# agentmorris/MegaDetector

Hardware: AMD Instinct MI355X
Metric: images/sec (whole node) MDv5a @1280px batch inference (higher is better)
Workload: dtype bf16

## Files before the change

### megadetector_amd/csrc/conv_v5c.cpp

```cpp

#include <algorithm>
#include <cstdlib>
#include <type_traits>

#include "mdhip_internal.h"

namespace mdhip {
namespace MDHIP_ST {

namespace {

typedef __attribute__((ext_vector_type(4))) float f32x4;
typedef __attribute__((address_space(3))) char lds_char;

[[maybe_unused]] constexpr unsigned kOOB = 0x80000000u;
[[maybe_unused]] constexpr int kNumRecords = 0x7fffffff;

__device__ __forceinline__ float silu_f32(float x) {
    return x * __builtin_amdgcn_rcpf(1.0f + __expf(-x));
}

constexpr int kPixB = 160;
constexpr int c80_run_bytes(int bm) { return ((bm + 2) * kPixB + 1023) & ~1023; }
constexpr int kW1Bytes = 9 * 80 * 32;
constexpr int c80_zero_bytes(int fm) { return ((15 + fm * 16 + 2) * kPixB + 32 + 255) & ~255; }
constexpr int c80_lds_bytes(int bm, int wm) { return 4 * c80_run_bytes(bm) + kW1Bytes + c80_zero_bytes(bm / (16 * wm)) + 320 + 1024; }
constexpr int c80f_lds_bytes(int bm, int wm) { return c80_lds_bytes(bm, wm) + 80 * 192 + 320; }
constexpr int c80_blocks(int bm, int wm) { return 163840 / c80_lds_bytes(bm, wm) >= 2 && wm == 1 ? 2 : 1; }

}

#define MDHIP_DMA16(rsrc, lptr, voff, soff) \
    __builtin_amdgcn_raw_ptr_buffer_load_lds((rsrc), (lptr), 16, (voff), (soff), 0, 0)

template <int BM, int WM>
__global__ void __launch_bounds__(WM * 5 * 64, c80_blocks(BM, WM))
conv_c80_kernel(const ConvArgs p) {
#if defined(__HIP_DEVICE_COMPILE__)
    constexpr int kNWc = WM * 5;
    constexpr int FM = BM / (16 * WM);
    constexpr int RUNB = c80_run_bytes(BM), PIECES = RUNB / 1024, NP = (PIECES + kNWc - 1) / kNWc;
    constexpr int W1_OFF = 4 * RUNB, ZERO_OFF = W1_OFF + kW1Bytes, BIAS_OFF = ZERO_OFF + c80_zero_bytes(FM);
    constexpr int SCRATCH_OFF = BIAS_OFF + 320;

    extern __shared__ __attribute__((aligned(16))) char smem_generic[];
    lds_char* const smem = (lds_char*)smem_generic;
    const int tid = threadIdx.x;
    const int lane = tid & 63;
    const int wave = __builtin_amdgcn_readfirstlane(tid >> 6);
    const int wm = wave / 5, wn = wave - 5 * wm;
    const int m15 = lane & 15, kb = lane >> 4;

    const int strips = p.tiles_n, segs = p.tiles_per_xcd, seg_rows = p.m_streams, total = p.tiles_m;
    const int xcd = blockIdx.x & 7, slot = blockIdx.x >> 3, slots = gridDim.x >> 3;
    const int per_xcd = (total + 7) / 8;
    const int u_lo = xcd * per_xcd, u_hi = min(u_lo + per_xcd, total);
    if (u_lo + slot >= u_hi) return;

    for (int c = tid * 16; c < c80_zero_bytes(FM); c += kNWc * 64 * 16)
        *(__attribute__((address_space(3))) uint4*)(smem + ZERO_OFF + c) = make_uint4(0, 0, 0, 0);
    for (int c = tid; c < 80; c += kNWc * 64) *(__attribute__((address_space(3))) float*)(smem + BIAS_OFF + c * 4) = p.bias[c];
    for (int c = tid; c < 9 * 80 * 2; c += kNWc * 64) {
        const int t = c / 160, rem = c - t * 160, ch = rem >> 1, half = rem & 1;
        *(__attribute__((address_space(3))) uint4*)(smem + W1_OFF + c * 16) =
            *(const uint4*)(p.wgt4 + (size_t)ch * p.k_pad4 + (9 + t) * 64 + half * 8);
    }
    frag8_t wreg[9][2];
#pragma unroll
    for (int t = 0; t < 9; ++t)
#pragma unroll
        for (int kk = 0; kk < 2; ++kk)
            wreg[t][kk] = *(const frag8_t*)(p.wgt4 + (size_t)(wn * 16 + m15) * p.k_pad4 + t * 64 + kk * 32 + kb * 8);
    const f32x4 bias4 = {p.bias[wn * 16 + kb * 4], p.bias[wn * 16 + kb * 4 + 1], p.bias[wn * 16 + kb * 4 + 2],
                         p.bias[wn * 16 + kb * 4 + 3]};

    int l_px[NP];
    unsigned l_off[NP], l_dst[NP];
#pragma unroll
    for (int k = 0; k < NP; ++k) {
        const int pc = wave + kNWc * k;
        const int g = pc * 64 + lane;
        const int px = g / 10, c16 = g - px * 10;
        l_px[k] = (pc < PIECES && px < BM + 2) ? px : 0x40000000;
        l_off[k] = (unsigned)((px * p.ld_in + c16 * 8) * 2);
        l_dst[k] = pc < PIECES ? (unsigned)(pc * 1024) : (unsigned)(SCRATCH_OFF - 0);
    }
    __amdgpu_buffer_rsrc_t in_rsrc, res_rsrc, out_rsrc;
    const int img_in_bytes = p.HoWo * p.ld_in * 2, img_out_bytes = p.HoWo * p.ld_out * 2, img_res_bytes = p.HoWo * p.ld_res * 2;
    int x0 = 0;
    auto issue_row = [&](int iy) __attribute__((always_inline)) {
        const unsigned sl = (unsigned)(((iy + 1) & 3) * RUNB);
        const bool row_ok = (unsigned)iy < (unsigned)p.H;
        const unsigned row_term = (unsigned)((iy * p.W + x0 - 1) * p.ld_in * 2);
#pragma unroll
        for (int k = 0; k < NP; ++k) {
            const bool ok = row_ok && (unsigned)(x0 - 1 + l_px[k]) < (unsigned)p.W;
            MDHIP_DMA16(in_rsrc, smem + (l_dst[k] >= (unsigned)SCRATCH_OFF ? l_dst[k] : sl + l_dst[k]), ok ? row_term + l_off[k] : kOOB, 0);
        }
    };

    const unsigned lane_a = (unsigned)((wm * (BM / WM) + m15) * kPixB + kb * 16);
    const unsigned lane_a1 = kb < 2 ? lane_a + 128u : 0xffffffffu;
    const unsigned lane_z = (unsigned)(ZERO_OFF + m15 * kPixB + (kb & 1) * 16);
    const unsigned lane_w1 = kb < 2 ? (unsigned)(W1_OFF + (wn * 16 + m15) * 32 + kb * 16) : (unsigned)ZERO_OFF;
    const unsigned lane_w1_step = kb < 2 ? 80u * 32u : 0u;

    f32x4 acc[FM];
#pragma unroll
    for (int i = 0; i < FM; ++i) acc[i] = f32x4{0.f, 0.f, 0.f, 0.f};

    bool first = true;
    for (int u = u_lo + slot; u < u_hi; u += slots) {
        const int xs = u % strips;
        const int t2 = u / strips;
        const int sg = t2 % segs, b = t2 / segs;
        x0 = xs * BM;
        const int y_lo = sg * seg_rows, y_hi = min(y_lo + seg_rows, p.H);
        in_rsrc = __builtin_amdgcn_make_buffer_rsrc((void*)(p.in + (size_t)b * p.HoWo * p.ld_in), 0, img_in_bytes, 0x00020000);
        out_rsrc = __builtin_amdgcn_make_buffer_rsrc((void*)((char*)p.out + (size_t)b * img_out_bytes), 0, img_out_bytes, 0x00020000);
        if (p.res)
            res_rsrc = __builtin_amdgcn_make_buffer_rsrc((void*)(p.res + (size_t)b * p.HoWo * p.ld_res), 0, img_res_bytes, 0x00020000);
        if (!first) __builtin_amdgcn_s_barrier();
        issue_row(y_lo - 1);
        issue_row(y_lo);
        issue_row(y_lo + 1);
        const int xw = x0 + wm * (BM / WM) + m15;
        for (int y = y_lo; y < y_hi; ++y) {
            if (first || y == y_lo) asm volatile("s_waitcnt vmcnt(0) lgkmcnt(0)" ::: "memory");
            else asm volatile("s_waitcnt vmcnt(%0)" ::"n"(FM) : "memory");
            first = false;
            __builtin_amdgcn_s_barrier();
            if (y + 1 < y_hi) issue_row(y + 2);
            typedef __attribute__((ext_vector_type(2))) unsigned u32x2;
            u32x2 rres[FM];
            if (p.res) {
#pragma unroll
                for (int i = 0; i < FM; ++i) {
                    const int x = xw + i * 16;
                    const unsigned off = x < p.W ? (unsigned)(((y * p.W + x) * p.ld_res + wn * 16 + kb * 4) * 2) : kOOB;
                    rres[i] = __builtin_amdgcn_raw_buffer_load_b64(res_rsrc, off, 0, 0);
                }
            }
            unsigned rb[3], rb1[3];
#pragma unroll
            for (int r = 0; r < 3; ++r) {
                const unsigned s0 = (unsigned)(((y + r) & 3) * RUNB);
                rb[r] = s0 + lane_a;
                rb1[r] = kb < 2 ? s0 + lane_a1 : lane_z;
            }
#pragma unroll
            for (int hs = 0; hs < 27; ++hs) {
                frag8_t xa[FM], w;
                if (hs < 18) {
                    const int t = hs >> 1, kk = hs & 1, r = t / 3, s = t - 3 * r;
#pragma unroll
                    for (int i = 0; i < FM; ++i)
                        xa[i] = *(const __attribute__((address_space(3))) frag8_t*)(smem + rb[r] + (i * 16 + s) * kPixB + kk * 64);
                    w = wreg[t][kk];
                } else {
                    const int t = hs - 18, r = t / 3, s = t - 3 * r;
#pragma unroll
                    for (int i = 0; i < FM; ++i)
                        xa[i] = *(const __attribute__((address_space(3))) frag8_t*)(smem + rb1[r] + (i * 16 + s) * kPixB);
                    w = *(const __attribute__((address_space(3))) frag8_t*)(smem + lane_w1 + t * lane_w1_step);
                }
#pragma unroll
                for (int i = 0; i < FM; ++i) acc[i] = MDHIP_MFMA(w, xa[i], acc[i]);
            }
#pragma unroll
            for (int i = 0; i < FM; ++i) {
                float v[4];
                mdhip_bias4(acc[i], bias4, v);
                if (p.act) mdhip_silu4(v);
                acc[i] = f32x4{0.f, 0.f, 0.f, 0.f};
                if (p.res) {
                    v[0] += st_unpack((uint16_t)(rres[i][0] & 0xffff));
                    v[1] += st_unpack((uint16_t)(rres[i][0] >> 16));
                    v[2] += st_unpack((uint16_t)(rres[i][1] & 0xffff));
                    v[3] += st_unpack((uint16_t)(rres[i][1] >> 16));
                }
                const u32x2 d = {st_pack2(v[0], v[1]), st_pack2(v[2], v[3])};
                const int x = xw + i * 16;
                const unsigned off = x < p.W ? (unsigned)(((y * p.W + x) * p.ld_out + wn * 16 + kb * 4) * 2) : kOOB;
                __builtin_amdgcn_raw_buffer_store_b64(d, out_rsrc, off, 0, 0);
            }
        }
    }
#endif
}

template <int BM, int WM>
__global__ void __launch_bounds__(WM * 5 * 64, 1)
conv_c80f_kernel(const ConvArgs p) {
#if defined(__HIP_DEVICE_COMPILE__)
    constexpr int kNWc = WM * 5;
    constexpr int FM = BM / (16 * WM);
    constexpr int RUNB = c80_run_bytes(BM), PIECES = RUNB / 1024, NP = (PIECES + kNWc - 1) / kNWc;
    constexpr int STAGE_OFF = 3 * RUNB;
    constexpr int W1_OFF = 4 * RUNB, ZERO_OFF = W1_OFF + kW1Bytes, BIAS_OFF = ZERO_OFF + c80_zero_bytes(FM);
    constexpr int SCRATCH_OFF = BIAS_OFF + 320;
    constexpr int WPRE_OFF = SCRATCH_OFF + 1024;
    constexpr int BPRE_OFF = WPRE_OFF + 80 * 192;
    constexpr int TF = (BM + 2 + 15) / 16;
    constexpr int TFW = (TF + WM - 1) / WM;
    static_assert(((TFW - 1) * 16 + 15) * kPixB + 16 <= c80_zero_bytes(FM) + 0, "zero region covers the conversion's immediates");

    extern __shared__ __attribute__((aligned(16))) char smem_generic[];
    lds_char* const smem = (lds_char*)smem_generic;
    const int tid = threadIdx.x;
    const int lane = tid & 63;
    const int wave = __builtin_amdgcn_readfirstlane(tid >> 6);
    const int wm = wave / 5, wn = wave - 5 * wm;
    const int m15 = lane & 15, kb = lane >> 4;

    const int strips = p.tiles_n, segs = p.tiles_per_xcd, seg_rows = p.m_streams, total = p.tiles_m;
    const int xcd = blockIdx.x & 7, slot = blockIdx.x >> 3, slots = gridDim.x >> 3;
    const int per_xcd = (total + 7) / 8;
    const int u_lo = xcd * per_xcd, u_hi = min(u_lo + per_xcd, total);
    if (u_lo + slot >= u_hi) return;

    for (int c = tid * 16; c < c80_zero_bytes(FM); c += kNWc * 64 * 16)
        *(__attribute__((address_space(3))) uint4*)(smem + ZERO_OFF + c) = make_uint4(0, 0, 0, 0);
    for (int c = tid; c < 9 * 80 * 2; c += kNWc * 64) {
        const int t = c / 160, rem = c - t * 160, ch = rem >> 1, half = rem & 1;
        *(__attribute__((address_space(3))) uint4*)(smem + W1_OFF + c * 16) =
            *(const uint4*)(p.wgt4 + (size_t)ch * p.k_pad4 + (9 + t) * 64 + half * 8);
    }
    frag8_t wreg[9][2];
#pragma unroll
    for (int t = 0; t < 9; ++t)
#pragma unroll
        for (int kk = 0; kk < 2; ++kk)
            wreg[t][kk] = *(const frag8_t*)(p.wgt4 + (size_t)(wn * 16 + m15) * p.k_pad4 + t * 64 + kk * 32 + kb * 8);
    for (int c = tid; c < 80 * 12; c += kNWc * 64) {
        const int ch = c / 12, q = c - ch * 12;
        *(__attribute__((address_space(3))) uint4*)(smem + WPRE_OFF + c * 16) = *(const uint4*)(p.wgt_pre + (size_t)ch * p.k_pad_pre + q * 8);
    }
    for (int c = tid; c < 80; c += kNWc * 64) *(__attribute__((address_space(3))) float*)(smem + BPRE_OFF + c * 4) = p.bias_pre[c];
    const unsigned lane_wp = (unsigned)(WPRE_OFF + (wn * 16 + m15) * 192 + kb * 16);
    const f32x4 bias4 = {p.bias[wn * 16 + kb * 4], p.bias[wn * 16 + kb * 4 + 1], p.bias[wn * 16 + kb * 4 + 2],
                         p.bias[wn * 16 + kb * 4 + 3]};

    __amdgpu_buffer_rsrc_t in_rsrc, res_rsrc, out_rsrc;
    const int img_in_bytes = p.HoWo * p.ld_in * 2, img_out_bytes = p.HoWo * p.ld_out * 2, img_res_bytes = p.HoWo * p.ld_res * 2;
    int x0 = 0;
    auto issue_row = [&](int iy) __attribute__((always_inline)) {
        const bool row_ok = (unsigned)iy < (unsigned)p.H;
        const unsigned row_term = (unsigned)((iy * p.W + x0 - 1) * p.ld_in * 2);
#pragma unroll
        for (int k = 0; k < NP; ++k) {
            const int pc = wave + kNWc * k;
            const int g = pc * 64 + lane;
            const int px = g / 10, c16 = g - px * 10;
            const bool ok = row_ok && pc < PIECES && px < BM + 2 && (unsigned)(x0 - 1 + px) < (unsigned)p.W;
            MDHIP_DMA16(in_rsrc, smem + (pc < PIECES ? STAGE_OFF + pc * 1024 : SCRATCH_OFF),
                        ok ? row_term + (unsigned)((px * p.ld_in + c16 * 8) * 2) : kOOB, 0);
        }
    };

    const unsigned lane_a = (unsigned)((wm * (BM / WM) + m15) * kPixB + kb * 16);
    const unsigned lane_a1 = kb < 2 ? lane_a + 128u : 0xffffffffu;
    const unsigned lane_z = (unsigned)(ZERO_OFF + m15 * kPixB + (kb & 1) * 16);
    const unsigned lane_w1 = kb < 2 ? (unsigned)(W1_OFF + (wn * 16 + m15) * 32 + kb * 16) : (unsigned)ZERO_OFF;
    const unsigned lane_w1_step = kb < 2 ? 80u * 32u : 0u;
    const unsigned lane_x = (unsigned)(STAGE_OFF + (wm * TFW * 16 + m15) * kPixB + kb * 16);
    const unsigned lane_x2 = kb < 2 ? lane_x + 128u : lane_z;
    const unsigned lane_t = (unsigned)((wm * TFW * 16 + m15) * kPixB + (wn * 16 + kb * 4) * 2);

    f32x4 acc[FM];
#pragma unroll
    for (int i = 0; i < FM; ++i) acc[i] = f32x4{0.f, 0.f, 0.f, 0.f};

    auto convert = [&](int iy, int ts) __attribute__((always_inline)) {
        const bool row_ok = (unsigned)iy < (unsigned)p.H;
        frag8_t wp[3];
#pragma unroll
        for (int t = 0; t < 3; ++t) wp[t] = *(const __attribute__((address_space(3))) frag8_t*)(smem + lane_wp + t * 64);
        const f32x4 bpre4 = *(const __attribute__((address_space(3))) f32x4*)(smem + BPRE_OFF + (wn * 16 + kb * 4) * 4);
#pragma unroll
        for (int f = 0; f < TFW; ++f) {
            if (wm * TFW + f < TF) {
                f32x4 c = {0.f, 0.f, 0.f, 0.f};
#pragma unroll
                for (int t = 0; t < 3; ++t) {
                    const frag8_t xf = *(const __attribute__((address_space(3))) frag8_t*)(smem + (t < 2 ? lane_x + t * 64 : lane_x2) + f * 16 * kPixB);
                    c = MDHIP_MFMA(wp[t], xf, c);
                }
                const int px = (wm * TFW + f) * 16 + m15;
                const bool ok = row_ok && px < BM + 2 && (unsigned)(x0 - 1 + px) < (unsigned)p.W;
                float v[4];
                mdhip_bias4(c, bpre4, v);
                mdhip_silu4(v);
                uint2 d;
                d.x = ok ? st_pack2(v[0], v[1]) : 0u;
                d.y = ok ? st_pack2(v[2], v[3]) : 0u;
                if (px < BM + 2)
                    *(__attribute__((address_space(3))) uint2*)(smem + ts * RUNB + lane_t + f * 16 * kPixB) = d;
            }
        }
    };

    bool first = true;
    for (int u = u_lo + slot; u < u_hi; u += slots) {
        const int xs = u % strips;
        const int t2 = u / strips;
        const int sg = t2 % segs, b = t2 / segs;
        x0 = xs * BM;
        const int y_lo = sg * seg_rows, y_hi = min(y_lo + seg_rows, p.H);
        in_rsrc = __builtin_amdgcn_make_buffer_rsrc((void*)(p.in + (size_t)b * p.HoWo * p.ld_in), 0, img_in_bytes, 0x00020000);
        out_rsrc = __builtin_amdgcn_make_buffer_rsrc((void*)((char*)p.out + (size_t)b * img_out_bytes), 0, img_out_bytes, 0x00020000);
        if (p.res)
            res_rsrc = __builtin_amdgcn_make_buffer_rsrc((void*)(p.res + (size_t)b * p.HoWo * p.ld_res), 0, img_res_bytes, 0x00020000);
        for (int k = 0; k < 3; ++k) {
            if (!first || k > 0) __builtin_amdgcn_s_barrier();
            first = false;
            issue_row(y_lo - 1 + k);
            asm volatile("s_waitcnt vmcnt(0) lgkmcnt(0)" ::: "memory");
            __builtin_amdgcn_s_barrier();
            convert(y_lo - 1 + k, k);
        }
        asm volatile("s_waitcnt lgkmcnt(0)" ::: "memory");
        __builtin_amdgcn_s_barrier();
        if (y_lo + 1 < y_hi) issue_row(y_lo + 2);
        const int xw = x0 + wm * (BM / WM) + m15;
        int s0 = 0;
        for (int y = y_lo; y < y_hi; ++y) {
            typedef __attribute__((ext_vector_type(2))) unsigned u32x2;
            u32x2 rres[FM];
            if (p.res) {
#pragma unroll
                for (int i = 0; i < FM; ++i) {
                    const int x = xw + i * 16;
                    const unsigned off = x < p.W ? (unsigned)(((y * p.W + x) * p.ld_res + wn * 16 + kb * 4) * 2) : kOOB;
                    rres[i] = __builtin_amdgcn_raw_buffer_load_b64(res_rsrc, off, 0, 0);
                }
            }
            unsigned rb[3], rb1[3];
#pragma unroll
            for (int r = 0; r < 3; ++r) {
                int sl = s0 + r;
                sl = sl >= 3 ? sl - 3 : sl;
                rb[r] = (unsigned)(sl * RUNB) + lane_a;
                rb1[r] = kb < 2 ? (unsigned)(sl * RUNB) + lane_a1 : lane_z;
            }
#pragma unroll
            for (int hs = 0; hs < 27; ++hs) {
                frag8_t xa[FM], w;
                if (hs < 18) {
                    const int t = hs >> 1, kk = hs & 1, r = t / 3, s = t - 3 * r;
#pragma unroll
                    for (int i = 0; i < FM; ++i)
                        xa[i] = *(const __attribute__((address_space(3))) frag8_t*)(smem + rb[r] + (i * 16 + s) * kPixB + kk * 64);
                    w = wreg[t][kk];
                } else {
                    const int t = hs - 18, r = t / 3, s = t - 3 * r;
#pragma unroll
                    for (int i = 0; i < FM; ++i)
                        xa[i] = *(const __attribute__((address_space(3))) frag8_t*)(smem + rb1[r] + (i * 16 + s) * kPixB);
                    w = *(const __attribute__((address_space(3))) frag8_t*)(smem + lane_w1 + t * lane_w1_step);
                }
#pragma unroll
                for (int i = 0; i < FM; ++i) acc[i] = MDHIP_MFMA(w, xa[i], acc[i]);
            }
#pragma unroll
            for (int i = 0; i < FM; ++i) {
                float v[4];
                mdhip_bias4(acc[i], bias4, v);
                if (p.act) mdhip_silu4(v);
                acc[i] = f32x4{0.f, 0.f, 0.f, 0.f};
                if (p.res) {
                    v[0] += st_unpack((uint16_t)(rres[i][0] & 0xffff));
                    v[1] += st_unpack((uint16_t)(rres[i][0] >> 16));
                    v[2] += st_unpack((uint16_t)(rres[i][1] & 0xffff));
                    v[3] += st_unpack((uint16_t)(rres[i][1] >> 16));
                }
                const u32x2 d = {st_pack2(v[0], v[1]), st_pack2(v[2], v[3])};
                const int x = xw + i * 16;
                const unsigned off = x < p.W ? (unsigned)(((y * p.W + x) * p.ld_out + wn * 16 + kb * 4) * 2) : kOOB;
                __builtin_amdgcn_raw_buffer_store_b64(d, out_rsrc, off, 0, 0);
            }
            if (y + 1 < y_hi) {
                asm volatile("s_waitcnt vmcnt(%0) lgkmcnt(0)" ::"n"(FM) : "memory");
                __builtin_amdgcn_s_barrier();
                convert(y + 2, s0);
                asm volatile("s_waitcnt lgkmcnt(0)" ::: "memory");
                __builtin_amdgcn_s_barrier();
                if (y + 2 < y_hi) issue_row(y + 3);
                s0 = s0 == 2 ? 0 : s0 + 1;
            }
        }
    }
#endif
}

constexpr int kD_BM = 64, kD_RW = 4, kD_RUNB = c80_run_bytes(kD_BM), kD_RING = kD_RW + 2;
constexpr int kD_STAGE_OFF = kD_RING * kD_RUNB, kD_W1_OFF = kD_STAGE_OFF + kD_RW * kD_RUNB, kD_ZERO_OFF = kD_W1_OFF + kW1Bytes;
constexpr int kD_WPRE_OFF = kD_ZERO_OFF + 256, kD_BPRE_OFF = kD_WPRE_OFF + 80 * 192, kD_LDS = kD_BPRE_OFF + 320;
static_assert(kD_LDS <= 163840, "LDS of the four-row fused bottleneck");
constexpr int kD_NB = 2, kD_RL = 4;

template <int PROF = 0, int NB = 4, int RL = 3>
__global__ void __launch_bounds__(640, 1)
conv_c80d_kernel(const ConvArgs p) {
#if defined(__HIP_DEVICE_COMPILE__)
    constexpr int BM = kD_BM, RW = kD_RW, RUNB = kD_RUNB, NRING = kD_RING, FMW = 2;
    constexpr int PIECES = RUNB / 1024, NP = (PIECES + 9) / 10;
    constexpr int STAGE_OFF = kD_STAGE_OFF, W1_OFF = kD_W1_OFF, ZERO_OFF = kD_ZERO_OFF, WPRE_OFF = kD_WPRE_OFF, BPRE_OFF = kD_BPRE_OFF;
    constexpr int TF = (BM + 2 + 15) / 16;
    static_assert(RUNB % 1024 == 0 && (BM + 2) * kPixB <= RUNB, "row slot");

    extern __shared__ __attribute__((aligned(16))) char smem_generic[];
    lds_char* const smem = (lds_char*)smem_generic;
    const int tid = threadIdx.x;
    const int lane = tid & 63;
    const int wave = __builtin_amdgcn_readfirstlane(tid >> 6);
    const int g = wave / 5, wn = wave - 5 * g;
    const int m15 = lane & 15, kb = lane >> 4;

    const int strips = p.tiles_n, segs = p.tiles_per_xcd, seg_rows = p.m_streams, total = p.tiles_m;
    const int xcd = blockIdx.x & 7, slot = blockIdx.x >> 3, slots = gridDim.x >> 3;
    const int per_xcd = (total + 7) / 8;
    const int u_lo = xcd * per_xcd, u_hi = min(u_lo + per_xcd, total);
    if (u_lo + slot >= u_hi) return;

    for (int c = tid * 16; c < W1_OFF; c += 640 * 16)
        *(__attribute__((address_space(3))) uint4*)(smem + c) = make_uint4(0, 0, 0, 0);
    if (tid < 16) *(__attribute__((address_space(3))) uint4*)(smem + ZERO_OFF + tid * 16) = make_uint4(0, 0, 0, 0);
    for (int c = tid; c < 9 * 80 * 2; c += 640) {
        const int t = c / 160, rem = c - t * 160, ch = rem >> 1, half = rem & 1;
        *(__attribute__((address_space(3))) uint4*)(smem + W1_OFF + c * 16) =
            *(const uint4*)(p.wgt4 + (size_t)ch * p.k_pad4 + (9 + t) * 64 + half * 8);
    }
    for (int c = tid; c < 80 * 12; c += 640) {
        const int ch = c / 12, q = c - ch * 12;
        *(__attribute__((address_space(3))) uint4*)(smem + WPRE_OFF + c * 16) = *(const uint4*)(p.wgt_pre + (size_t)ch * p.k_pad_pre + q * 8);
    }
    for (int c = tid; c < 80; c += 640) *(__attribute__((address_space(3))) float*)(smem + BPRE_OFF + c * 4) = p.bias_pre[c];
    frag8_t wreg[9][2];
#pragma unroll
    for (int t = 0; t < 9; ++t)
#pragma unroll
        for (int kk = 0; kk < 2; ++kk)
            wreg[t][kk] = *(const frag8_t*)(p.wgt4 + (size_t)(wn * 16 + m15) * p.k_pad4 + t * 64 + kk * 32 + kb * 8);
    const f32x4 bias4 = {p.bias[wn * 16 + kb * 4], p.bias[wn * 16 + kb * 4 + 1], p.bias[wn * 16 + kb * 4 + 2],
                         p.bias[wn * 16 + kb * 4 + 3]};

    __amdgpu_buffer_rsrc_t in_rsrc, res_rsrc, out_rsrc;
    const int img_in_bytes = p.HoWo * p.ld_in * 2, img_out_bytes = p.HoWo * p.ld_out * 2, img_res_bytes = p.HoWo * p.ld_res * 2;
    int x0 = 0;
    auto issue_row = [&](int iy, int st) __attribute__((always_inline)) {
        const bool row_ok = (unsigned)iy < (unsigned)p.H;
        const unsigned row_term = (unsigned)((iy * p.W + x0 - 1) * p.ld_in * 2);
        int lane_o = lane;
        asm volatile("" : "+v"(lane_o));
#pragma unroll
        for (int k = 0; k < NP; ++k) {
            const int pc = wave + 10 * k;
            if (pc >= PIECES) continue;
            const int gch = pc * 64 + lane_o;
            const int px = gch / 10, c16 = gch - px * 10;
            const bool ok = row_ok && px < BM + 2 && (unsigned)(x0 - 1 + px) < (unsigned)p.W;
            MDHIP_DMA16(in_rsrc, smem + STAGE_OFF + st * RUNB + pc * 1024, ok ? row_term + (unsigned)((px * p.ld_in + c16 * 8) * 2) : kOOB, 0);
        }
    };

    const unsigned lane_a = (unsigned)((g * (BM / 2) + m15) * kPixB + kb * 16);
    const unsigned lane_w1 = kb < 2 ? (unsigned)(W1_OFF + (wn * 16 + m15) * 32 + kb * 16) : (unsigned)ZERO_OFF;
    const unsigned lane_w1_step = kb < 2 ? 80u * 32u : 0u;

    f32x4 acc[RW][FMW];
#pragma unroll
    for (int rr = 0; rr < RW; ++rr)
#pragma unroll
        for (int i = 0; i < FMW; ++i) acc[rr][i] = f32x4{0.f, 0.f, 0.f, 0.f};

    auto convert = [&](int iy, int st, int ts, int cf) __attribute__((always_inline)) {
        const bool row_ok = (unsigned)iy < (unsigned)p.H;
        int lane_o = lane;
        asm volatile("" : "+v"(lane_o));
        const int m15 = lane_o & 15, kb = lane_o >> 4;
        const unsigned lane_x = (unsigned)(STAGE_OFF + m15 * kPixB + kb * 16);
        const unsigned lane_t = (unsigned)(m15 * kPixB + (cf * 16 + kb * 4) * 2);
        const unsigned lane_wp = (unsigned)(WPRE_OFF + (cf * 16 + m15) * 192 + kb * 16);
        frag8_t wp[3];
#pragma unroll
        for (int t = 0; t < 3; ++t) wp[t] = *(const __attribute__((address_space(3))) frag8_t*)(smem + lane_wp + t * 64);
        const f32x4 bpre4 = *(const __attribute__((address_space(3))) f32x4*)(smem + BPRE_OFF + (cf * 16 + kb * 4) * 4);
        frag8_t xf[TF][3];
#pragma unroll
        for (int f = 0; f < TF; ++f)
#pragma unroll
            for (int t = 0; t < 3; ++t)
                xf[f][t] = *(const __attribute__((address_space(3))) frag8_t*)(smem + lane_x + st * RUNB + f * 16 * kPixB + t * 64);
        f32x4 c[TF];
#pragma unroll
        for (int f = 0; f < TF; ++f) c[f] = f32x4{0.f, 0.f, 0.f, 0.f};
#pragma unroll
        for (int t = 0; t < 3; ++t)
#pragma unroll
            for (int f = 0; f < TF; ++f) c[f] = MDHIP_MFMA(wp[t], xf[f][t], c[f]);
        uint2 d[TF];
#pragma unroll
        for (int f = 0; f < TF; ++f) {
            const int px = f * 16 + m15;
            const bool ok = row_ok && px < BM + 2 && (unsigned)(x0 - 1 + px) < (unsigned)p.W;
            float v[4];
            mdhip_bias4(c[f], bpre4, v);
            mdhip_silu4(v);
            d[f].x = ok ? st_pack2(v[0], v[1]) : 0u;
            d[f].y = ok ? st_pack2(v[2], v[3]) : 0u;
        }
#pragma unroll
        for (int f = 0; f < TF; ++f) {
            const int px = f * 16 + m15;
            if (px < BM + 2)
                *(__attribute__((address_space(3))) uint2*)(smem + ts * RUNB + lane_t + f * 16 * kPixB) = d[f];
        }
    };
    auto ring_slot = [&](int i) __attribute__((always_inline)) -> int { return i >= NRING ? i - NRING : i; };
    constexpr unsigned long long kTask0 = 0ull | (2ull << 5) | (4ull << 10) | (7ull << 15) | (10ull << 20) | (12ull << 25) | (14ull << 30) |
                                          (16ull << 35) | (18ull << 40) | (19ull << 45) | (20ull << 50);
    static_assert(RW == 4, "task table of the conversion");
    const int task_lo = (int)((kTask0 >> (5 * wave)) & 31), task_hi = (int)((kTask0 >> (5 * wave + 5)) & 31);
    auto convert_rows = [&](int y_first, int slot0) __attribute__((always_inline)) {
#pragma unroll
        for (int k = 0; k < 3; ++k) {
            const int id = task_lo + k;
            if (id < task_hi) {
                const int row = id / 5, cf = id - 5 * row;
                convert(y_first + row, row, ring_slot(slot0 + row), cf);
            }
        }
    };
    unsigned long long t_acc[6] = {0, 0, 0, 0, 0, 0}, t_prev = 0, n_tiles = 0;
    auto stamp = [&](int k) __attribute__((always_inline)) {
        if constexpr (PROF != 0) {
            const unsigned long long t = __builtin_amdgcn_s_memtime();
            t_acc[k] += t - t_prev;
            t_prev = t;
        }
    };
    if constexpr (PROF != 0) t_prev = __builtin_amdgcn_s_memtime();

    bool first = true;
    for (int u = u_lo + slot; u < u_hi; u += slots) {
        const int xs = u % strips;
        const int t2 = u / strips;
        const int sg = t2 % segs, b = t2 / segs;
        x0 = xs * BM;
        const int y_lo = sg * seg_rows, y_hi = min(y_lo + seg_rows, p.H);
        in_rsrc = __builtin_amdgcn_make_buffer_rsrc((void*)(p.in + (size_t)b * p.HoWo * p.ld_in), 0, img_in_bytes, 0x00020000);
        out_rsrc = __builtin_amdgcn_make_buffer_rsrc((void*)((char*)p.out + (size_t)b * img_out_bytes), 0, img_out_bytes, 0x00020000);
        res_rsrc = __builtin_amdgcn_make_buffer_rsrc((void*)(p.res ? p.res + (size_t)b * p.HoWo * p.ld_res : p.in), 0,
                                                     p.res ? img_res_bytes : 0, 0x00020000);
        if (first) {
            asm volatile("s_waitcnt lgkmcnt(0)" ::: "memory");
            __builtin_amdgcn_s_barrier();
            first = false;
        }
#pragma unroll
        for (int k = 0; k < RW; ++k) issue_row(y_lo - 1 + k, k);
        asm volatile("s_waitcnt vmcnt(0) lgkmcnt(0)" ::: "memory");
        __builtin_amdgcn_s_barrier();
        convert_rows(y_lo - 1, 0);
        asm volatile("s_waitcnt lgkmcnt(0)" ::: "memory");
        __builtin_amdgcn_s_barrier();
        issue_row(y_lo - 1 + RW, 0);
        issue_row(y_lo + RW, 1);
        asm volatile("s_waitcnt vmcnt(0) lgkmcnt(0)" ::: "memory");
        __builtin_amdgcn_s_barrier();
        convert(y_lo - 1 + RW + g, g, RW + g, wn);
        asm volatile("s_waitcnt lgkmcnt(0)" ::: "memory");
        __builtin_amdgcn_s_barrier();
        if (y_lo + RW < y_hi) {
#pragma unroll
            for (int k = 0; k < RW; ++k) issue_row(y_lo + RW + 1 + k, k);
        }
        int s0 = 0;
        stamp(5);
        for (int y = y_lo; y < y_hi; y += RW) {
            typedef __attribute__((ext_vector_type(2))) unsigned u32x2;
            u32x2 rres[RW][FMW];
            ++n_tiles;
            constexpr int NS1 = (RW + 2) * 6, NS2 = (RW + 2) * 3, NS = NS1 + NS2;
            frag8_t xq[NB][FMW];
            frag8_t w1[9];
            auto load_x = [&](int st) __attribute__((always_inline)) {
                if (st < NS1) {
                    const int qi = st / 6, s = (st % 6) >> 1, kk = st & 1;
                    const unsigned base = (unsigned)(ring_slot(s0 + qi) * RUNB) + lane_a;
#pragma unroll
                    for (int i = 0; i < FMW; ++i)
                        xq[st % NB][i] = *(const __attribute__((address_space(3))) frag8_t*)(smem + base + (i * 16 + s) * kPixB + kk * 64);
                } else {
                    const int qi = (st - NS1) / 3, s = (st - NS1) % 3;
                    const unsigned base = (unsigned)(ring_slot(s0 + qi) * RUNB) + lane_a + 128u;
#pragma unroll
                    for (int i = 0; i < FMW; ++i)
                        xq[st % NB][i] = *(const __attribute__((address_space(3))) frag8_t*)(smem + base + (i * 16 + s) * kPixB);
                }
            };
#pragma unroll
            for (int st = 0; st < NB - 1; ++st) load_x(st);
#pragma unroll
            for (int st = 0; st < NS1; ++st) {
                load_x(st + NB - 1);
                __builtin_amdgcn_sched_barrier(0);
                const int qi = st / 6, s = (st % 6) >> 1, kk = st & 1;
#pragma unroll
                for (int rr = 0; rr < RW; ++rr) {
                    const int r = qi - rr;
                    if (r < 0 || r > 2) continue;
#pragma unroll
                    for (int i = 0; i < FMW; ++i) acc[rr][i] = MDHIP_MFMA(wreg[r * 3 + s][kk], xq[st % NB][i], acc[rr][i]);
                }
                __builtin_amdgcn_sched_barrier(0);
            }
            stamp(0);
#pragma unroll
            for (int t = 0; t < 9; ++t)
                w1[t] = *(const __attribute__((address_space(3))) frag8_t*)(smem + lane_w1 + t * lane_w1_step);
            {
                int lane_o = lane;
                asm volatile("" : "+v"(lane_o));
                const int xw = x0 + g * (BM / 2) + (lane_o & 15), kb = lane_o >> 4;
#pragma unroll
                for (int rr = 0; rr < RW; ++rr)
#pragma unroll
                    for (int i = 0; i < FMW; ++i) {
                        const int x = xw + i * 16;
                        const unsigned off = (x < p.W && y + rr < y_hi) ? (unsigned)((((y + rr) * p.W + x) * p.ld_res + wn * 16 + kb * 4) * 2) : kOOB;
                        rres[rr][i] = __builtin_amdgcn_raw_buffer_load_b64(res_rsrc, off, 0, 0);
                    }
            }
            auto epilogue_frag = [&](int rr, int i) __attribute__((always_inline)) {
                int lane_e = lane;
                asm volatile("" : "+v"(lane_e));
                const int xw = x0 + g * (BM / 2) + (lane_e & 15), kb = lane_e >> 4;
                float v[4];
                mdhip_bias4(acc[rr][i], bias4, v);
                if (p.act) mdhip_silu4(v);
                acc[rr][i] = f32x4{0.f, 0.f, 0.f, 0.f};
                v[0] += st_unpack((uint16_t)(rres[rr][i][0] & 0xffff));
                v[1] += st_unpack((uint16_t)(rres[rr][i][0] >> 16));
                v[2] += st_unpack((uint16_t)(rres[rr][i][1] & 0xffff));
                v[3] += st_unpack((uint16_t)(rres[rr][i][1] >> 16));
                const u32x2 d = {st_pack2(v[0], v[1]), st_pack2(v[2], v[3])};
                const int x = xw + i * 16;
                const unsigned off = (x < p.W && y + rr < y_hi) ? (unsigned)((((y + rr) * p.W + x) * p.ld_out + wn * 16 + kb * 4) * 2) : kOOB;
                __builtin_amdgcn_raw_buffer_store_b64(d, out_rsrc, off, 0, 0);
            };
#pragma unroll
            for (int st = NS1; st < NS; ++st) {
                if (st + NB - 1 < NS) load_x(st + NB - 1);
                __builtin_amdgcn_sched_barrier(0);
                const int qi = (st - NS1) / 3, s = (st - NS1) % 3;
#pragma unroll
                for (int rr = 0; rr < RW; ++rr) {
                    const int r = qi - rr;
                    if (r < 0 || r > 2) continue;
#pragma unroll
                    for (int i = 0; i < FMW; ++i) acc[rr][i] = MDHIP_MFMA(w1[r * 3 + s], xq[st % NB][i], acc[rr][i]);
                }
                if (qi >= 3 && s < FMW) epilogue_frag(qi - 3, s);
                __builtin_amdgcn_sched_barrier(0);
            }
            stamp(1);
#pragma unroll
            for (int i = 0; i < FMW; ++i) epilogue_frag(RW - 1, i);
            {
                asm volatile("" ::: "memory");
                int lane_w = lane;
                asm volatile("" : "+v"(lane_w));
                const uint16_t* wrow = p.wgt4 + (size_t)(wn * 16 + (lane_w & 15)) * p.k_pad4 + (lane_w >> 4) * 8;
#pragma unroll
                for (int t = RL; t < 9; ++t)
#pragma unroll
                    for (int kk = 0; kk < 2; ++kk) wreg[t][kk] = *(const frag8_t*)(wrow + t * 64 + kk * 32);
            }
            stamp(2);
            if (y + RW < y_hi) {
                asm volatile("s_waitcnt vmcnt(%0) lgkmcnt(0)" ::"n"(RW * FMW + 2 * (9 - RL)) : "memory");
                __builtin_amdgcn_s_barrier();
                stamp(3);
                convert_rows(y + RW + 1, s0);
                stamp(4);
                asm volatile("s_waitcnt lgkmcnt(0)" ::: "memory");
                __builtin_amdgcn_s_barrier();
                if (y + 2 * RW < y_hi) {
#pragma unroll
                    for (int k = 0; k < RW; ++k) issue_row(y + 2 * RW + 1 + k, k);
                }
                s0 = ring_slot(s0 + RW);
                stamp(5);
            }
        }
    }
    if constexpr (PROF != 0) {
        if (lane == 0 && p.dbg) {
            unsigned long long* d = (unsigned long long*)p.dbg + ((size_t)blockIdx.x * 10 + wave) * 8;
            for (int k = 0; k < 6; ++k) d[k] = t_acc[k];
            d[6] = n_tiles;
            d[7] = (unsigned long long)__builtin_amdgcn_s_getreg(((6 - 1) << 11) | (0 << 6) | 4) | 0x100;
        }
    }
#endif
}

#define MDHIP_CONV5C_CFGS(X) \
    X(0, 160, 2)             \
    X(1, 128, 2)
constexpr int kCfgR4 = 2;

static const ConvCfg g_cfgs5c[] = {
#define X(id, bm, wm) {bm, 80, (wm) * 5 * 64, (size_t)c80_lds_bytes(bm, wm), c80_blocks(bm, wm), "v5:strip" #bm "x80/" #wm "x5"},
    MDHIP_CONV5C_CFGS(X)
#undef X
    {kD_BM, 80, 640, (size_t)kD_LDS, 1, "v5:strip64x80/2x5/r4"},
    {kD_BM, 80, 640, (size_t)kD_LDS, 1, "dev:strip64x80/2x5/r4/nb2rl4"},
    {kD_BM, 80, 640, (size_t)kD_LDS, 1, "dev:strip64x80/2x5/r4/nb2rl3"},
    {kD_BM, 80, 640, (size_t)kD_LDS, 1, "dev:strip64x80/2x5/r4/nb2rl5"},
    {kD_BM, 80, 640, (size_t)kD_LDS, 1, "dev:strip64x80/2x5/r4/nb3rl3"},
    {kD_BM, 80, 640, (size_t)kD_LDS, 1, "dev:strip64x80/2x5/r4/nb4rl3"},
};


int conv5c_num_cfgs() { return (int)(sizeof(g_cfgs5c) / sizeof(g_cfgs5c[0])); }
const ConvCfg& conv5c_cfg(int i) { return g_cfgs5c[i]; }

hipError_t conv5c_init() {
    hipError_t e = hipSuccess;
#define X(id, bm, wm)                                                                            \
    if (e == hipSuccess)                                                                         \
        e = hipFuncSetAttribute((const void*)conv_c80_kernel<bm, wm>, hipFuncAttributeMaxDynamicSharedMemorySize, \
                                (int)g_cfgs5c[id].lds_bytes);                                       \
    if (e == hipSuccess)                                                                         \
        e = hipFuncSetAttribute((const void*)conv_c80f_kernel<bm, wm>, hipFuncAttributeMaxDynamicSharedMemorySize, \
                                c80f_lds_bytes(bm, wm));

    MDHIP_CONV5C_CFGS(X)
#undef X
#define MDHIP_C80D_VARIANTS(X) X(0, 1, 2, 4) X(1, 1, 2, 3) X(2, 1, 2, 5) X(3, 1, 3, 3) X(4, 1, 4, 3)
    if (e == hipSuccess) e = hipFuncSetAttribute((const void*)conv_c80d_kernel<0, kD_NB, kD_RL>, hipFuncAttributeMaxDynamicSharedMemorySize, kD_LDS);
#define X(id, prof, nb, rl) \
    if (e == hipSuccess) e = hipFuncSetAttribute((const void*)conv_c80d_kernel<prof, nb, rl>, hipFuncAttributeMaxDynamicSharedMemorySize, kD_LDS);
    MDHIP_C80D_VARIANTS(X)
#undef X
    return e;
}

bool conv5c_supports(int cfg, const ConvArgs& a) {
    if (a.wgt_pre != nullptr && (a.bias_pre == nullptr || a.k_pad_pre < 96 || (const void*)a.in == (const void*)a.out || a.act != 1))
        return false;
    if (cfg > kCfgR4 && (a.dbg == nullptr || a.wgt_pre == nullptr)) return false;
    return cfg >= 0 && cfg < conv5c_num_cfgs() && !a.out_f32 && !a.out_f8 && !a.in_f8 && a.C8 == 10 && a.groups == 2 &&
           a.N == 80 && a.n_rows == 80 && (long long)a.HoWo * a.ld_in * 2 < 0x3fffffffLL &&
           (long long)a.HoWo * a.ld_out * 2 < 0x3fffffffLL && (a.res == nullptr || (long long)a.HoWo * a.ld_res * 2 < 0x3fffffffLL);
}

hipError_t conv5c_launch(int cfg, const ConvArgs& a, hipStream_t s) {
    const int dev = cfg > kCfgR4 ? cfg - kCfgR4 - 1 : -1;
    if (dev >= 0) cfg = kCfgR4;
    if (cfg == kCfgR4 && !a.wgt_pre) cfg = 0;
    const ConvCfg& c = g_cfgs5c[cfg];
    ConvArgs p = a;
    const int n_img = a.M / a.HoWo;
    if (cfg == kCfgR4) {
        const int strips = (a.W + kD_BM - 1) / kD_BM;
        int best_rows = 4;
        double best_cost = 1e30;
        for (int sr = 4; sr <= ((a.H + 3) / 4) * 4; sr += 4) {
            const long long units = (long long)n_img * strips * ((a.H + sr - 1) / sr);
            const double cost = (double)((units + 255) / 256) * (sr + 3.0);
            if (cost < best_cost) { best_cost = cost; best_rows = sr; }
        }
        p.tiles_n = strips;
        p.tiles_per_xcd = (a.H + best_rows - 1) / best_rows;
        p.m_streams = best_rows;
        p.tiles_m = n_img * p.tiles_per_xcd * strips;
        const int slots = std::max(1, std::min(32, (p.tiles_m + 7) / 8));
        const dim3 grid_d((unsigned)(8 * slots));
        switch (dev) {
#define X(id, prof, nb, rl) case id: hipLaunchKernelGGL((conv_c80d_kernel<prof, nb, rl>), grid_d, dim3(640), kD_LDS, s, p); break;
            MDHIP_C80D_VARIANTS(X)
#undef X
            default: hipLaunchKernelGGL((conv_c80d_kernel<0, kD_NB, kD_RL>), grid_d, dim3(640), kD_LDS, s, p); break;
        }
        return hipGetLastError();
    }
    const int strips = (a.W + c.bm - 1) / c.bm;
    const int wgs = 256 * c.blocks_per_cu;
    int seg_rows = (int)std::max(8LL, std::min<long long>(a.H, ((long long)n_img * strips * a.H + 4 * wgs - 1) / (4 * wgs)));
    const int segs = (a.H + seg_rows - 1) / seg_rows;
    p.tiles_n = strips;
    p.tiles_per_xcd = segs;
    p.m_streams = seg_rows;
    p.tiles_m = n_img * segs * strips;
    const int slots = std::max(1, std::min(32 * c.blocks_per_cu, (p.tiles_m + 7) / 8));
    const dim3 grid((unsigned)(8 * slots));
    switch (cfg) {
#define X(id, bm, wm)                                                                             \
    case id:                                                                                      \
        if (a.wgt_pre) hipLaunchKernelGGL((conv_c80f_kernel<bm, wm>), grid, dim3((wm) * 5 * 64), c80f_lds_bytes(bm, wm), s, p); \
        else hipLaunchKernelGGL((conv_c80_kernel<bm, wm>), grid, dim3((wm) * 5 * 64), c.lds_bytes, s, p); \
        break;
        MDHIP_CONV5C_CFGS(X)
#undef X
    }
    return hipGetLastError();
}

}
}
```

Measured before the change: 1101.

## Interleave pre-conv conversion of next rows into the 3x3 MFMA pass via slot pool

The kernel replaces the separate staging buffer and ring with a pool of NRING+RW row slots. Incoming raw rows are DMA'd directly into future pool slots, and the 1x1 pre-conv conversion (bias+SiLU) for the next row band is spread as per-chunk work inside the first pass of the 3x3 MFMA loop. This removes the serialized convert phase and one of its barriers between tiles, hiding conversion behind main-loop MFMAs. The cost is higher register and LDS pressure and a more complex schedule. It also adds an env override for the segment row count.

```diff
diff --git a/megadetector_amd/csrc/conv_v5c.cpp b/megadetector_amd/csrc/conv_v5c.cpp
--- a/megadetector_amd/csrc/conv_v5c.cpp
+++ b/megadetector_amd/csrc/conv_v5c.cpp
@@ -398,14 +398,15 @@
 constexpr int kD_WPRE_OFF = kD_ZERO_OFF + 256, kD_BPRE_OFF = kD_WPRE_OFF + 80 * 192, kD_LDS = kD_BPRE_OFF + 320;
 static_assert(kD_LDS <= 163840, "LDS of the four-row fused bottleneck");
 constexpr int kD_NB = 2, kD_RL = 4;
+constexpr int kD_CV0 = 15;
 
 template <int PROF = 0, int NB = 4, int RL = 3>
 __global__ void __launch_bounds__(640, 1)
 conv_c80d_kernel(const ConvArgs p) {
 #if defined(__HIP_DEVICE_COMPILE__)
-    constexpr int BM = kD_BM, RW = kD_RW, RUNB = kD_RUNB, NRING = kD_RING, FMW = 2;
+    constexpr int BM = kD_BM, RW = kD_RW, RUNB = kD_RUNB, NRING = kD_RING, NPOOL = kD_RING + kD_RW, FMW = 2, CV0 = kD_CV0;
     constexpr int PIECES = RUNB / 1024, NP = (PIECES + 9) / 10;
-    constexpr int STAGE_OFF = kD_STAGE_OFF, W1_OFF = kD_W1_OFF, ZERO_OFF = kD_ZERO_OFF, WPRE_OFF = kD_WPRE_OFF, BPRE_OFF = kD_BPRE_OFF;
+    constexpr int W1_OFF = kD_W1_OFF, ZERO_OFF = kD_ZERO_OFF, WPRE_OFF = kD_WPRE_OFF, BPRE_OFF = kD_BPRE_OFF;
     constexpr int TF = (BM + 2 + 15) / 16;
     static_assert(RUNB % 1024 == 0 && (BM + 2) * kPixB <= RUNB, "row slot");
 
@@ -448,7 +449,8 @@
     __amdgpu_buffer_rsrc_t in_rsrc, res_rsrc, out_rsrc;
     const int img_in_bytes = p.HoWo * p.ld_in * 2, img_out_bytes = p.HoWo * p.ld_out * 2, img_res_bytes = p.HoWo * p.ld_res * 2;
     int x0 = 0;
-    auto issue_row = [&](int iy, int st) __attribute__((always_inline)) {
+    auto pool_slot = [&](int i) __attribute__((always_inline)) -> int { return i >= NPOOL ? i - NPOOL : i; };
+    auto issue_row = [&](int iy, int sl) __attribute__((always_inline)) {
         const bool row_ok = (unsigned)iy < (unsigned)p.H;
         const unsigned row_term = (unsigned)((iy * p.W + x0 - 1) * p.ld_in * 2);
         int lane_o = lane;
@@ -460,13 +462,11 @@
             const int gch = pc * 64 + lane_o;
             const int px = gch / 10, c16 = gch - px * 10;
             const bool ok = row_ok && px < BM + 2 && (unsigned)(x0 - 1 + px) < (unsigned)p.W;
-            MDHIP_DMA16(in_rsrc, smem + STAGE_OFF + st * RUNB + pc * 1024, ok ? row_term + (unsigned)((px * p.ld_in + c16 * 8) * 2) : kOOB, 0);
+            MDHIP_DMA16(in_rsrc, smem + sl * RUNB + pc * 1024, ok ? row_term + (unsigned)((px * p.ld_in + c16 * 8) * 2) : kOOB, 0);
         }
     };
 
     const unsigned lane_a = (unsigned)((g * (BM / 2) + m15) * kPixB + kb * 16);
-    const unsigned lane_w1 = kb < 2 ? (unsigned)(W1_OFF + (wn * 16 + m15) * 32 + kb * 16) : (unsigned)ZERO_OFF;
-    const unsigned lane_w1_step = kb < 2 ? 80u * 32u : 0u;
 
     f32x4 acc[RW][FMW];
 #pragma unroll
@@ -474,64 +474,58 @@
 #pragma unroll
         for (int i = 0; i < FMW; ++i) acc[rr][i] = f32x4{0.f, 0.f, 0.f, 0.f};
 
-    auto convert = [&](int iy, int st, int ts, int cf) __attribute__((always_inline)) {
-        const bool row_ok = (unsigned)iy < (unsigned)p.H;
+    frag8_t cx[3];
+    auto cv_load = [&](int sl, int f) __attribute__((always_inline)) {
+        int lane_o = lane;
+        asm volatile("" : "+v"(lane_o));
+        const unsigned a = (unsigned)(sl * RUNB + f * 16 * kPixB) + (unsigned)((lane_o & 15) * kPixB + (lane_o >> 4) * 16);
+#pragma unroll
+        for (int t = 0; t < 3; ++t) cx[t] = *(const __attribute__((address_space(3))) frag8_t*)(smem + a + t * 64);
+    };
+    auto cv_frag = [&](int iy, int f, int cf, int m15, int kb) __attribute__((always_inline)) -> uint2 {
+        const unsigned lane_wp = (unsigned)(WPRE_OFF + (cf * 16 + m15) * 192 + kb * 16);
+        f32x4 c = {0.f, 0.f, 0.f, 0.f};
+#pragma unroll
+        for (int t = 0; t < 3; ++t)
+            c = MDHIP_MFMA(*(const __attribute__((address_space(3))) frag8_t*)(smem + lane_wp + t * 64), cx[t], c);
+        const f32x4 bpre4 = *(const __attribute__((address_space(3))) f32x4*)(smem + BPRE_OFF + (cf * 16 + kb * 4) * 4);
+        const int px = f * 16 + m15;
+        const bool ok = (unsigned)iy < (unsigned)p.H && px < BM + 2 && (unsigned)(x0 - 1 + px) < (unsigned)p.W;
+        float v[4];
+        mdhip_bias4(c, bpre4, v);
+        mdhip_silu4(v);
+        uint2 d;
+        d.x = ok ? st_pack2(v[0], v[1]) : 0u;
+        d.y = ok ? st_pack2(v[2], v[3]) : 0u;
+        return d;
+    };
+    auto cv_chunk = [&](int iy, int sl, int f, int cf) __attribute__((always_inline)) {
         int lane_o = lane;
         asm volatile("" : "+v"(lane_o));
         const int m15 = lane_o & 15, kb = lane_o >> 4;
-        const unsigned lane_x = (unsigned)(STAGE_OFF + m15 * kPixB + kb * 16);
-        const unsigned lane_t = (unsigned)(m15 * kPixB + (cf * 16 + kb * 4) * 2);
-        const unsigned lane_wp = (unsigned)(WPRE_OFF + (cf * 16 + m15) * 192 + kb * 16);
-        frag8_t wp[3];
-#pragma unroll
-        for (int t = 0; t < 3; ++t) wp[t] = *(const __attribute__((address_space(3))) frag8_t*)(smem + lane_wp + t * 64);
-        const f32x4 bpre4 = *(const __attribute__((address_space(3))) f32x4*)(smem + BPRE_OFF + (cf * 16 + kb * 4) * 4);
-        frag8_t xf[TF][3];
-#pragma unroll
-        for (int f = 0; f < TF; ++f)
-#pragma unroll
-            for (int t = 0; t < 3; ++t)
-                xf[f][t] = *(const __attribute__((address_space(3))) frag8_t*)(smem + lane_x + st * RUNB + f * 16 * kPixB + t * 64);
-        f32x4 c[TF];
-#pragma unroll
-        for (int f = 0; f < TF; ++f) c[f] = f32x4{0.f, 0.f, 0.f, 0.f};
-#pragma unroll
-        for (int t = 0; t < 3; ++t)
-#pragma unroll
-            for (int f = 0; f < TF; ++f) c[f] = MDHIP_MFMA(wp[t], xf[f][t], c[f]);
-        uint2 d[TF];
-#pragma unroll
-        for (int f = 0; f < TF; ++f) {
-            const int px = f * 16 + m15;
-            const bool ok = row_ok && px < BM + 2 && (unsigned)(x0 - 1 + px) < (unsigned)p.W;
-            float v[4];
-            mdhip_bias4(c[f], bpre4, v);
-            mdhip_silu4(v);
-            d[f].x = ok ? st_pack2(v[0], v[1]) : 0u;
-            d[f].y = ok ? st_pack2(v[2], v[3]) : 0u;
-        }
-#pragma unroll
-        for (int f = 0; f < TF; ++f) {
-            const int px = f * 16 + m15;
+        const uint2 d = cv_frag(iy, f, cf, m15, kb);
+        const int px = f * 16 + m15;
+        if (px < BM + 2)
+            *(__attribute__((address_space(3))) uint2*)(smem + sl * RUNB + px * kPixB + (cf * 16 + kb * 4) * 2) = d;
+    };
+    auto cv_task = [&](int iy, int sl, int f) __attribute__((always_inline)) {
+        int lane_o = lane;
+        asm volatile("" : "+v"(lane_o));
+        const int m15 = lane_o & 15, kb = lane_o >> 4;
+        cv_load(sl, f);
+        uint2 d[5];
+#pragma unroll
+        for (int cf = 0; cf < 5; ++cf) d[cf] = cv_frag(iy, f, cf, m15, kb);
+        const int px = f * 16 + m15;
+#pragma unroll
+        for (int cf = 0; cf < 5; ++cf)
             if (px < BM + 2)
-                *(__attribute__((address_space(3))) uint2*)(smem + ts * RUNB + lane_t + f * 16 * kPixB) = d[f];
-        }
+                *(__attribute__((address_space(3))) uint2*)(smem + sl * RUNB + px * kPixB + (cf * 16 + kb * 4) * 2) = d[cf];
     };
-    auto ring_slot = [&](int i) __attribute__((always_inline)) -> int { return i >= NRING ? i - NRING : i; };
     constexpr unsigned long long kTask0 = 0ull | (2ull << 5) | (4ull << 10) | (7ull << 15) | (10ull << 20) | (12ull << 25) | (14ull << 30) |
                                           (16ull << 35) | (18ull << 40) | (19ull << 45) | (20ull << 50);
-    static_assert(RW == 4, "task table of the conversion");
+    static_assert(RW == 4 && TF == 5, "task table of the conversion");
     const int task_lo = (int)((kTask0 >> (5 * wave)) & 31), task_hi = (int)((kTask0 >> (5 * wave + 5)) & 31);
-    auto convert_rows = [&](int y_first, int slot0) __attribute__((always_inline)) {
-#pragma unroll
-        for (int k = 0; k < 3; ++k) {
-            const int id = task_lo + k;
-            if (id < task_hi) {
-                const int row = id / 5, cf = id - 5 * row;
-                convert(y_first + row, row, ring_slot(slot0 + row), cf);
-            }
-        }
-    };
     unsigned long long t_acc[6] = {0, 0, 0, 0, 0, 0}, t_prev = 0, n_tiles = 0;
     auto stamp = [&](int k) __attribute__((always_inline)) {
         if constexpr (PROF != 0) {
@@ -542,7 +536,6 @@
     };
     if constexpr (PROF != 0) t_prev = __builtin_amdgcn_s_memtime();
 
-    bool first = true;
     for (int u = u_lo + slot; u < u_hi; u += slots) {
         const int xs = u % strips;
         const int t2 = u / strips;
@@ -553,48 +546,45 @@
         out_rsrc = __builtin_amdgcn_make_buffer_rsrc((void*)((char*)p.out + (size_t)b * img_out_bytes), 0, img_out_bytes, 0x00020000);
         res_rsrc = __builtin_amdgcn_make_buffer_rsrc((void*)(p.res ? p.res + (size_t)b * p.HoWo * p.ld_res : p.in), 0,
                                                      p.res ? img_res_bytes : 0, 0x00020000);
-        if (first) {
-            asm volatile("s_waitcnt lgkmcnt(0)" ::: "memory");
-            __builtin_amdgcn_s_barrier();
-            first = false;
-        }
-#pragma unroll
-        for (int k = 0; k < RW; ++k) issue_row(y_lo - 1 + k, k);
+        asm volatile("s_waitcnt lgkmcnt(0)" ::: "memory");
+        __builtin_amdgcn_s_barrier();
+#pragma unroll
+        for (int k = 0; k < NRING; ++k) issue_row(y_lo - 1 + k, k);
         asm volatile("s_waitcnt vmcnt(0) lgkmcnt(0)" ::: "memory");
         __builtin_amdgcn_s_barrier();
-        convert_rows(y_lo - 1, 0);
+        if (y_lo + RW < y_hi) {
+#pragma unroll
+            for (int k = 0; k < RW; ++k) issue_row(y_lo + RW + 1 + k, NRING + k);
+        }
+#pragma unroll
+        for (int k = 0; k < 3; ++k) {
+            const int id = wave + 10 * k, row = id / TF, f = id - TF * row;
+            cv_task(y_lo - 1 + row, row, f);
+        }
         asm volatile("s_waitcnt lgkmcnt(0)" ::: "memory");
         __builtin_amdgcn_s_barrier();
-        issue_row(y_lo - 1 + RW, 0);
-        issue_row(y_lo + RW, 1);
-        asm volatile("s_waitcnt vmcnt(0) lgkmcnt(0)" ::: "memory");
-        __builtin_amdgcn_s_barrier();
-        convert(y_lo - 1 + RW + g, g, RW + g, wn);
-        asm volatile("s_waitcnt lgkmcnt(0)" ::: "memory");
-        __builtin_amdgcn_s_barrier();
-        if (y_lo + RW < y_hi) {
-#pragma unroll
-            for (int k = 0; k < RW; ++k) issue_row(y_lo + RW + 1 + k, k);
-        }
         int s0 = 0;
         stamp(5);
         for (int y = y_lo; y < y_hi; y += RW) {
             typedef __attribute__((ext_vector_type(2))) unsigned u32x2;
             u32x2 rres[RW][FMW];
             ++n_tiles;
+            const bool have_next = y + RW < y_hi;
+            const int my_tasks = have_next ? task_hi - task_lo : 0;
             constexpr int NS1 = (RW + 2) * 6, NS2 = (RW + 2) * 3, NS = NS1 + NS2;
+            static_assert(CV0 + 15 <= NS1, "the conversion's chunks sit in pass 1");
             frag8_t xq[NB][FMW];
             frag8_t w1[9];
             auto load_x = [&](int st) __attribute__((always_inline)) {
                 if (st < NS1) {
                     const int qi = st / 6, s = (st % 6) >> 1, kk = st & 1;
-                    const unsigned base = (unsigned)(ring_slot(s0 + qi) * RUNB) + lane_a;
+                    const unsigned base = (unsigned)(pool_slot(s0 + qi) * RUNB) + lane_a;
 #pragma unroll
                     for (int i = 0; i < FMW; ++i)
                         xq[st % NB][i] = *(const __attribute__((address_space(3))) frag8_t*)(smem + base + (i * 16 + s) * kPixB + kk * 64);
                 } else {
                     const int qi = (st - NS1) / 3, s = (st - NS1) % 3;
-                    const unsigned base = (unsigned)(ring_slot(s0 + qi) * RUNB) + lane_a + 128u;
+                    const unsigned base = (unsigned)(pool_slot(s0 + qi) * RUNB) + lane_a + 128u;
 #pragma unroll
                     for (int i = 0; i < FMW; ++i)
                         xq[st % NB][i] = *(const __attribute__((address_space(3))) frag8_t*)(smem + base + (i * 16 + s) * kPixB);
@@ -604,6 +594,14 @@
             for (int st = 0; st < NB - 1; ++st) load_x(st);
 #pragma unroll
             for (int st = 0; st < NS1; ++st) {
+                if (st == CV0) {
+                    stamp(0);
+                    if (have_next) {
+                        asm volatile("s_waitcnt vmcnt(0)" ::: "memory");
+                        __builtin_amdgcn_s_barrier();
+                    }
+                    stamp(1);
+                }
                 load_x(st + NB - 1);
                 __builtin_amdgcn_sched_barrier(0);
                 const int qi = st / 6, s = (st % 6) >> 1, kk = st & 1;
@@ -614,15 +612,29 @@
 #pragma unroll
                     for (int i = 0; i < FMW; ++i) acc[rr][i] = MDHIP_MFMA(wreg[r * 3 + s][kk], xq[st % NB][i], acc[rr][i]);
                 }
+                if (st >= CV0 && st < CV0 + 15) {
+                    const int k = (st - CV0) / 5, cf = (st - CV0) % 5;
+                    if (k < my_tasks) {
+                        const int id = task_lo + k, row = id / TF, f = id - TF * row;
+                        const int sl = pool_slot(s0 + NRING + row);
+                        if (cf == 0) cv_load(sl, f);
+                        cv_chunk(y + RW + 1 + row, sl, f, cf);
+                    }
+                }
                 __builtin_amdgcn_sched_barrier(0);
             }
-            stamp(0);
-#pragma unroll
-            for (int t = 0; t < 9; ++t)
-                w1[t] = *(const __attribute__((address_space(3))) frag8_t*)(smem + lane_w1 + t * lane_w1_step);
+            stamp(2);
             {
                 int lane_o = lane;
                 asm volatile("" : "+v"(lane_o));
+                {
+                    const int m15 = lane_o & 15, kb = lane_o >> 4;
+                    const unsigned lane_w1 = kb < 2 ? (unsigned)(W1_OFF + (wn * 16 + m15) * 32 + kb * 16) : (unsigned)ZERO_OFF;
+                    const unsigned lane_w1_step = kb < 2 ? 80u * 32u : 0u;
+#pragma unroll
+                    for (int t = 0; t < 9; ++t)
+                        w1[t] = *(const __attribute__((address_space(3))) frag8_t*)(smem + lane_w1 + t * lane_w1_step);
+                }
                 const int xw = x0 + g * (BM / 2) + (lane_o & 15), kb = lane_o >> 4;
 #pragma unroll
                 for (int rr = 0; rr < RW; ++rr)
@@ -665,7 +677,7 @@
                 if (qi >= 3 && s < FMW) epilogue_frag(qi - 3, s);
                 __builtin_amdgcn_sched_barrier(0);
             }
-            stamp(1);
+            stamp(3);
 #pragma unroll
             for (int i = 0; i < FMW; ++i) epilogue_frag(RW - 1, i);
             {
@@ -678,20 +690,15 @@
 #pragma unroll
                     for (int kk = 0; kk < 2; ++kk) wreg[t][kk] = *(const frag8_t*)(wrow + t * 64 + kk * 32);
             }
-            stamp(2);
-            if (y + RW < y_hi) {
-                asm volatile("s_waitcnt vmcnt(%0) lgkmcnt(0)" ::"n"(RW * FMW + 2 * (9 - RL)) : "memory");
-                __builtin_amdgcn_s_barrier();
-                stamp(3);
-                convert_rows(y + RW + 1, s0);
-                stamp(4);
+            stamp(4);
+            if (have_next) {
                 asm volatile("s_waitcnt lgkmcnt(0)" ::: "memory");
                 __builtin_amdgcn_s_barrier();
+                s0 = pool_slot(s0 + RW);
                 if (y + 2 * RW < y_hi) {
 #pragma unroll
-                    for (int k = 0; k < RW; ++k) issue_row(y + 2 * RW + 1 + k, k);
-                }
-                s0 = ring_slot(s0 + RW);
+                    for (int k = 0; k < RW; ++k) issue_row(y + 2 * RW + 1 + k, pool_slot(s0 + NRING + k));
+                }
                 stamp(5);
             }
         }
@@ -773,6 +780,10 @@
             const long long units = (long long)n_img * strips * ((a.H + sr - 1) / sr);
             const double cost = (double)((units + 255) / 256) * (sr + 3.0);
             if (cost < best_cost) { best_cost = cost; best_rows = sr; }
+        }
+        if (const char* e = getenv("MDHIP_C80_SEG_ROWS")) {
+            const int v = atoi(e);
+            if (v > 0) best_rows = std::min(v, a.H);
         }
         p.tiles_n = strips;
         p.tiles_per_xcd = (a.H + best_rows - 1) / best_rows;
```

Result: no change. 1095 (-0.6%).
